# Jackson-D-Taylor/PINT

Measured on AMD Instinct MI355X. Metric: GLS fits/sec, 68-PSR x 10k-TOA synthetic PTA (whole node), higher is better.
Workload: dtype f64+dd; 1 GPU; pta68x10k GLSFitter.fit_toas(maxiter=1) incl. noise realisations (the 68-pulsar PTA, LPT-sharded over 1 rank(s)); npsr=68, ntoas=10000, K_cols_max=178, launch=direct, pipelines=2, parallelism=pulsar shards x1 (LPT, no data-path collective)

## Files before the change

### pint_amd/csrc/pint_hip.hip

```cpp
#include <hip/hip_runtime.h>
#include <hip/hip_ext.h>
#include <string>
#include <vector>
#include <cstring>
#include <cstdio>
#include <algorithm>
#include <array>
#include <utility>
#include <cmath>
#include <cstdlib>
#include <map>
#include <type_traits>
#include <mutex>
#include <functional>
#include <chrono>
#include "physics.hpp"
#include "ensemble.hpp"

using namespace pint;

typedef double double4_t __attribute__((ext_vector_type(4)));

__device__ __forceinline__ void rot(double& c, double& s, double c1, double s1) {
    const double cn = c * c1 - s * s1;
// ... 66 lines not shown
    const int32_t* fdj_index;
    const uint64_t *fdjmask, *fdjdmmask;
    int o_pw, npw, o_wave, nwave, sifunc, nifunc;
    const double *ifx_hi, *ifx_lo, *ify;
    const int32_t* dm_cls;
    const double* dme0;
    int ndmcls;
};

struct InstDev {
    int psr;
    int n;
    int K;
    int Kp;
    long toff;
    long roff;
    long moff;
    long goff;
    long soff;
    long coff;
    long cvoff;
    long eoff;
    long epoff;
    long ooff;
    long sdoff;
    long ddoff;
    long vgoff;
    long vboff;
    long xwoff;
    int self;
    int nrb;
    long rb0;
    int neb;
    long eb0;
    const pint_spec_t* spec;
    const ColRun* runs;
    int ts;
    int nrun;
};

struct GramView {
    const double* Gp;
    int Kp;
    const int32_t* cmap;
    const double* Sd;
    const double* DD;
    __device__ __forceinline__ double operator()(int i, int j) const {
        if (!cmap) {
            if (i > j) { int t = i; i = j; j = t; }
            return Gp[(long)i * Kp + j];
        }
        int a = cmap[i], b = cmap[j];
        if (a >= 0 && b >= 0) {
            if (a > b) { int t = a; a = b; b = t; }
            return Gp[(long)a * Kp + b];
        }
        if (a < 0 && b < 0) return a == b ? DD[-a - 1] : 0.0;
        if (a < 0) return Sd[(long)(-a - 1) * Kp + b];
        return Sd[(long)(-b - 1) * Kp + a];
    }
};

__device__ __forceinline__ GramView gram_view(const PsrDev& Pd, const InstDev& I, const double* Gpart, bool cmp,
                                              const double* Sd, const double* DD) {
    GramView g;
    g.Gp = Gpart + I.goff;
// ... 2318 lines not shown
        part[(long)blockIdx.x * 512 + e] = (red[e] + red[512 + e]) + (red[1024 + e] + red[1536 + e]);
}

__global__ __launch_bounds__(256) void k_trig_sum(const TrigJob* __restrict__ jobs, const double* __restrict__ part) {
    __shared__ double T[512];
    const TrigJob J = jobs[blockIdx.x];
    for (int e = threadIdx.x; e < 512; e += 256) {
        double v = 0.0;
        for (int b = 0; b < J.nb; b++) v += part[(long)(J.b0 + b) * 512 + e];
        T[e] = v;
    }
    __syncthreads();
    const int m = threadIdx.x & 63, a = m & 7, b = m >> 3, kind = threadIdx.x >> 6;
    if (kind < 2 && (kind == 1 || J.trigU)) {
        const double* D = T + kind * 256;
        double* o = kind ? J.trigW : J.trigU;
        o[m] = D[a * 16 + b] - D[(8 + a) * 16 + 8 + b];
        o[VTRIG + m] = D[(8 + a) * 16 + b] + D[a * 16 + 8 + b];
    }
}

struct GredArgs {
    int nsplit, nparts, compact, vb;
    double* Gpart;
    double* colsq;
    const double* Sdp;
    const double* dmxv;
    double* Sd;
    double* DD;
    double* DCS;
    const double* BFp;
};

__device__ __forceinline__ void gred_bin(const InstDev& I, const PsrDev& Pd, const GredArgs& g, int a, int lane) {
    const int Kp = Pd.Kpd, Kc = Pd.Kd, r0 = Pd.red0c, nsplit = g.nsplit;
    const int SW = Kc + 3;
    const int cnt = Pd.dptr[a + 1] - Pd.dptr[a];
    const long lo = cnt > 0 ? Pd.didx[Pd.dptr[a]] : 0, hi = lo + cnt;
    long per = (I.n + nsplit - 1) / nsplit;
    per = (per + 3) / 4 * 4;
    const int q0 = (int)(lo / per), q1 = cnt > 0 ? (int)((hi - 1) / per) : q0 - 1;
    const double* part = g.Sdp + I.vgoff + (long)(a % Pd.vns) * SW;
    constexpr int GRB_R = 4;
    const bool vbp = g.vb && Pd.vb;
    double dcs[2][2 * GW][2];
    bool use[2 * GW];
    long doff[2 * GW];
#pragma unroll
    for (int k = 0; k < 2 * GW; k++) {
        const int q = q0 + k / GW, w = k % GW;
        const long s0_ = (long)q * per, s1_ = min((long)I.n, s0_ + per), len = s1_ - s0_;
        const long QV = (len + VCH - 1) / VCH * 16;
        const long w0 = s0_ + w * QV, w1 = min(s1_, w0 + QV);
        use[k] = q <= q1 && !(w0 >= w1 || hi <= w0 || lo >= w1);
        doff[k] = I.vboff + (((long)q * GW + w) * Pd.vns + a % Pd.vns) * 128;
    }
    double xr[GRB_R], sr[GRB_R];
#pragma unroll
    for (int u = 0; u < GRB_R; u++) {
        const long i = lo + lane + 64 * u;
        xr[u] = i < hi ? g.dmxv[I.ooff + i] : 0.0;
        sr[u] = i < hi ? Pd.isig[i] : 0.0;
    }
#pragma unroll
    for (int t = 0; t < 2; t++) {
        const int c = lane + 64 * t;
        const bool fc = vbp && c >= r0 && c < Kc;
        int e0 = 0, e1 = 0;
        if (fc) {
            const int h = (c - r0) >> 1, k = h + 1, a_ = k & 7, cc = k >> 3;
            const bool isin = ((c - r0) & 1) == 0;
            e0 = isin ? (8 + a_) * 8 + cc : a_ * 8 + cc;
            e1 = isin ? a_ * 8 + 4 + cc : (8 + a_) * 8 + 4 + cc;
        }
#pragma unroll
        for (int k = 0; k < 2 * GW; k++) {
            const bool ld = c <= Kc && (fc ? use[k] : (k % GW == 0 && q0 + k / GW <= q1));
            dcs[t][k][0] = ld ? (fc ? g.BFp[doff[k] + e0] : part[(long)(q0 + k / GW) * Pd.vns * SW + c]) : 0.0;
            dcs[t][k][1] = (ld && fc) ? g.BFp[doff[k] + e1] : 0.0;
        }
    }
#pragma unroll
    for (int t = 0; t < 2; t++) {
        const int c = lane + 64 * t;
        if (c > Kc) break;
        double v = 0.0;
        if (vbp && c >= r0 && c < Kc) {
            const bool isin = ((c - r0) & 1) == 0;
            const double sg = isin ? 1.0 : -1.0;
#pragma unroll
            for (int k = 0; k < 2 * GW; k++)
                if (use[k]) v += dcs[t][k][0] + sg * dcs[t][k][1];
            for (int q = q0 + 2; q <= q1; q++) {
                const int h = (c - r0) >> 1, kk = h + 1, a_ = kk & 7, cc = kk >> 3;
                const int e0 = isin ? (8 + a_) * 8 + cc : a_ * 8 + cc;
                const int e1 = isin ? a_ * 8 + 4 + cc : (8 + a_) * 8 + 4 + cc;
                const long s0_ = (long)q * per, s1_ = min((long)I.n, s0_ + per), len = s1_ - s0_;
                const long QV = (len + VCH - 1) / VCH * 16;
                for (int w = 0; w < GW; w++) {
                    const long w0 = s0_ + w * QV, w1 = min(s1_, w0 + QV);
                    if (w0 >= w1 || hi <= w0 || lo >= w1) continue;
                    const double* D = g.BFp + I.vboff + (((long)q * GW + w) * Pd.vns + a % Pd.vns) * 128;
                    v += D[e0] + sg * D[e1];
                }
            }
        } else {
#pragma unroll
            for (int k = 0; k < 2; k++)
                if (q0 + k <= q1) v += dcs[t][k * GW][0];
            for (int q = q0 + 2; q <= q1; q++) v += part[(long)q * Pd.vns * SW + c];
        }
        g.Sd[I.sdoff + (long)a * Kp + c] = v;
    }
    for (int c = lane + 128; c <= Kc; c += 64) {
        double v = 0.0;
        if (vbp && c >= r0 && c < Kc) {
            const int h = (c - r0) >> 1, k = h + 1, a_ = k & 7, cc = k >> 3;
            const bool isin = ((c - r0) & 1) == 0;
            const int e0 = isin ? (8 + a_) * 8 + cc : a_ * 8 + cc;
            const int e1 = isin ? a_ * 8 + 4 + cc : (8 + a_) * 8 + 4 + cc;
            const double sg = isin ? 1.0 : -1.0;
            for (int q = q0; q <= q1; q++) {
                const long s0_ = (long)q * per, s1_ = min((long)I.n, s0_ + per), len = s1_ - s0_;
                const long QV = (len + VCH - 1) / VCH * 16;
                for (int w = 0; w < GW; w++) {
                    const long w0 = s0_ + w * QV, w1 = min(s1_, w0 + QV);
                    if (w0 >= w1 || hi <= w0 || lo >= w1) continue;
                    const double* D = g.BFp + I.vboff + (((long)q * GW + w) * Pd.vns + a % Pd.vns) * 128;
                    v += D[e0] + sg * D[e1];
                }
            }
        } else {
            for (int q = q0; q <= q1; q++) v += part[(long)q * Pd.vns * SW + c];
        }
        g.Sd[I.sdoff + (long)a * Kp + c] = v;
    }
    double q2 = 0.0, qw = 0.0;
#pragma unroll
    for (int u = 0; u < GRB_R; u++) {
        if (lo + lane + 64 * u < hi) {
            const double xx = xr[u], xw = xx * sr[u];
            q2 += xx * xx;
            qw += xw * xw;
        }
    }
    for (long i = lo + lane + 64 * GRB_R; i < hi; i += 64) {
        const double xx = g.dmxv[I.ooff + i], xw = xx * Pd.isig[i];
        q2 += xx * xx;
        qw += xw * xw;
    }
    q2 = wave_sum(q2);
    qw = wave_sum(qw);
    if (lane == 0) {
        g.DCS[I.ddoff + a] = q2;
        g.DD[I.ddoff + a] = qw;
    }
}

__device__ __forceinline__ void gred_elem(const InstDev& I, const PsrDev& Pd, const GredArgs& g, long e) {
    const bool cmp = g.compact && Pd.dsplit;
    const bool vg = cmp && Pd.vg;
    const int Kp = cmp ? Pd.Kpd : I.Kp, Kc = cmp ? Pd.Kd : I.K;
    const int r0 = Pd.red0c;
    const long KK = (long)Kp * Kp;
    if (e < KK) {
        const int i = (int)(e / Kp), j = (int)(e % Kp);
        if (i <= j) {
            double* G = g.Gpart + I.goff;
            if (vg && (j > Kc)) {
                G[e] = 0.0;
            } else if (vg && i >= r0 && j < Kc) {
                const double* C = Pd.trigW;
                const double* Sn = C + VTRIG;
                const int ha = (i - r0) / 2 + 1, sa = (i - r0) & 1;
                const int hb = (j - r0) / 2 + 1, sb = (j - r0) & 1;
                const int dm = ha > hb ? ha - hb : hb - ha, sm = ha + hb;
                const double sd = ha >= hb ? Sn[ha - hb] : -Sn[hb - ha];
                double v;
                if (sa == 0 && sb == 0) v = 0.5 * (C[dm] - C[sm]);
                else if (sa == 1 && sb == 1) v = 0.5 * (C[dm] + C[sm]);
                else if (sa == 0) v = 0.5 * (Sn[sm] + sd);
                else v = 0.5 * (Sn[sm] - sd);
                G[e] = v;
            } else {
                double a[8] = {G[e], 0.0, 0.0, 0.0, 0.0, 0.0, 0.0, 0.0};
                int q = 1;
                for (; q + 32 <= g.nparts; q += 32) {
                    double t[32];
#pragma unroll
                    for (int u = 0; u < 32; u++) t[u] = G[(long)(q + u) * KK + e];
#pragma unroll
                    for (int u = 0; u < 32; u++) a[u & 7] += t[u];
                }
                {
                    const int rem = g.nparts - q;
                    double t[31];
#pragma unroll
                    for (int u = 0; u < 31; u++) t[u] = u < rem ? G[(long)(q + u) * KK + e] : 0.0;
#pragma unroll
                    for (int r = 0; r < 3; r++)
                        if (8 * r + 8 <= rem) {
#pragma unroll
                            for (int u = 0; u < 8; u++) a[u] += t[8 * r + u];
                        }
#pragma unroll
                    for (int u = 0; u < 31; u++)
                        if (u >= (rem & ~7) && u < rem) a[0] += t[u];
                }
                G[e] = ((a[0] + a[1]) + (a[2] + a[3])) + ((a[4] + a[5]) + (a[6] + a[7]));
            }
        }
    }
    if (e < Kc) {
        double* cs = g.colsq + (I.coff + e) * g.nsplit;
        if (vg && e >= r0) {
            const double* U = Pd.trigU;
            const int h = (int)(e - r0) / 2 + 1;
            cs[0] = 0.5 * (U[0] + (((e - r0) & 1) ? U[2 * h] : -U[2 * h]));
        } else {
            double a[4] = {cs[0], 0.0, 0.0, 0.0};
            int q = 1;
            for (; q + 32 <= g.nsplit; q += 32) {
                double t[32];
#pragma unroll
                for (int u = 0; u < 32; u++) t[u] = cs[q + u];
#pragma unroll
                for (int u = 0; u < 32; u++) a[u & 3] += t[u];
            }
            {
                const int rem = g.nsplit - q;
                double t[31];
#pragma unroll
                for (int u = 0; u < 31; u++) t[u] = u < rem ? cs[q + u] : 0.0;
#pragma unroll
                for (int r = 0; r < 7; r++)
                    if (4 * r + 4 <= rem) {
#pragma unroll
                        for (int u = 0; u < 4; u++) a[u] += t[4 * r + u];
                    }
#pragma unroll
                for (int u = 0; u < 31; u++)
                    if (u >= (rem & ~3) && u < rem) a[0] += t[u];
            }
            cs[0] = (a[0] + a[1]) + (a[2] + a[3]);
        }
    }
}

__global__ __launch_bounds__(256) void k_greduce(const PsrDev* __restrict__ psrs, const InstDev* __restrict__ insts,
                                                 int nbg, GredArgs g) {
    WgTimer wgt_(WGT_GRED);
    const InstDev I = insts[blockIdx.y];
    const PsrDev& Pd = psrs[I.psr];
    const bool vg = g.compact && Pd.dsplit && Pd.vg;
    if ((int)blockIdx.x >= nbg) {
        const int a = (blockIdx.x - nbg) * 4 + (threadIdx.x >> 6);
        if (!vg || a >= Pd.ndc) return;
        gred_bin(I, Pd, g, a, threadIdx.x & 63);
        return;
    }
    gred_elem(I, Pd, g, (long)blockIdx.x * blockDim.x + threadIdx.x);
}

__device__ __forceinline__ bool ones_virtual(const pint_spec_t& S) { return S.o_PHOFF >= 0 && !S.wb_noones; }

__global__ __launch_bounds__(64) void k_onesrow(const PsrDev* __restrict__ psrs, const InstDev* __restrict__ insts,
                                                const double* __restrict__ esum, const double* __restrict__ eD,
                                                const double* __restrict__ eW, const double* __restrict__ eC,
                                                int compact, const double* __restrict__ M, double* __restrict__ ones) {
    const InstDev I = insts[blockIdx.x];
    const PsrDev& Pd = psrs[I.psr];
    const pint_spec_t& S = *Pd.spec;
    if (!ones_virtual(S) || !(S.nred > 0 || Pd.nep > 0)) return;
    const bool cmp = compact && Pd.dsplit;
    const int R = 2 * S.nred, jd = 2 * S.dmn0;
    if (jd < R) {
        const int n = I.n;
        const double* Fb = M + I.moff + (long)(cmp ? Pd.red0c : S.ncol) * n;
        for (int j = jd; j < R; j++) {
            double acc = 0.0;
            for (int i = threadIdx.x; i < n; i += 64) {
                const double is = Pd.isig[i];
                acc += Fb[(long)j * n + i] * (is * is);
            }
            acc = wave_sum(acc);
            if (threadIdx.x == 0) {
                for (int e = 0; e < Pd.nep; e++) {
                    const double w = eW[I.epoff + e];
                    acc -= w * esum_col(Pd, I, esum, eC, cmp, e, S.ncol + j) / eD[I.epoff + e];
                }
                ones[I.coff + j] = acc;
            }
        }
    }
// ... 3002 lines not shown
    bool psrs_dirty = false;
    PsrDev* d_psrs = nullptr;
    int npsr_dev = 0;
    int ninst = 0;
    std::vector<InstDev> inst;
    InstDev* d_inst = nullptr;
    InstDev* d_inst_sorted = nullptr;
    InstDev* d_inst_sorted_c = nullptr;
    InstDev* d_inst_sorted_v = nullptr;
    bool sorted_alias[3] = {false, false, false};
    double* d_gridspec = nullptr;
    std::vector<KpGroup> kp_groups, kp_groups_c, kp_groups_v;
    int vgram = 1;
    int vbin = 1;
    int wbfit = 0;
    int gv_pair = 1;
    int maxn = 0;
    int max_ts = 0;
    int resid12 = 1;
    int prep_lanes = 1;
    int fuse_r2 = 1;
    bool r2_pending = false;
    int resid_path = 0;
    int eval_path = 0;
    int eval_kinds = 0;
    bool grid_valid = false;
    std::vector<double> grid_spec_host;
    int grid_psr = -1;
    std::vector<int32_t> points_toff;
    bool points_valid = false;
    struct EnsState* ens = nullptr;
    long grid_opts = 0;
    int small = 1;
    int schur = 1;
    int evalb_wpe = 3;
    int la_chol = 1;
    int solve_w8 = 1;
    int eval0_wpe = 1;
    int eval_wpe = 3;
    int n_vg = 0;
    bool any_dmx_rows = false;
    double *d_TSp = nullptr, *d_TS = nullptr;
    double* d_Sdp = nullptr;
    double* d_BFp = nullptr;
    int vb_on = 0;
    double* d_xw = nullptr;
    int cov_defer = 1;
    bool cov_pending = false;
    int cov_mode = 0;
    size_t cov_lds = 0;
    bool ic_valid = false;
    bool phases_valid = false;
    bool no_events = false;
    int timing_mask = 0xff;
    int timing_every = 1;
    long gram_calls = 0;
    static constexpr int NSLOT = PINT_NSLOT;
    hipGraph_t graph_s[NSLOT] = {};
    hipGraphExec_t graph_exec_s[NSLOT] = {};
    bool capturing = false;
    int* d_blk_inst = nullptr;
    int* d_blk_row0 = nullptr;
    int* d_rblk_inst = nullptr;
    double* d_rpart = nullptr;
    double* d_epart = nullptr;
    int efz = 0;
// ... 532 lines not shown
        return;
    }
    std::lock_guard<std::mutex> lk(g_stream_mu);
    g_stream_pool[role][device][g_stream_rank[s]] = s;
}

pint_ctx* pint_ctx_create(int device) {
    pint_ctx* ctx = new pint_ctx();
    ctx->device = device;
    if (hipSetDevice(device) != hipSuccess) {
        ctx->err = "hipSetDevice failed";
        return ctx;
    }
    {
        int ncu = 0;
        if (hipDeviceGetAttribute(&ncu, hipDeviceAttributeMultiprocessorCount, device) == hipSuccess && ncu > 0) ctx->ncu = ncu;
    }
    ctx->stream = stream_get(device, STREAM_KERNEL);
    ctx->cstream = stream_get(device, STREAM_COPY);
    const unsigned evf = hipEventDisableTiming |
                         ((getenv("PINT_EV_SYSTEM") && atoi(getenv("PINT_EV_SYSTEM"))) ? 0u : hipEventReleaseToDevice);
    hipEventCreateWithFlags(&ctx->ev_solved, evf);
    hipEventCreateWithFlags(&ctx->ev_copied, evf);
    hipEventCreateWithFlags(&ctx->ev_noise, evf);
    if (getenv("PINT_SERIAL") && atoi(getenv("PINT_SERIAL"))) ctx->sstream = ctx->stream;
    else ctx->sstream = stream_get(device, STREAM_SIDE);
    ctx->no_events = getenv("PINT_NO_EVENTS") && atoi(getenv("PINT_NO_EVENTS"));
    ctx->eval_merge = getenv("PINT_EVAL_MERGE") ? atoi(getenv("PINT_EVAL_MERGE")) : 3;
    ctx->vbin = getenv("PINT_VBIN") ? (atoi(getenv("PINT_VBIN")) ? 1 : 0) : 1;
    ctx->cov_defer = getenv("PINT_COV_DEFER") ? atoi(getenv("PINT_COV_DEFER")) : 1;
    ctx->eval_wpe = getenv("PINT_EVAL_WPE") ? atoi(getenv("PINT_EVAL_WPE")) : 3;
    ctx->gv_pair = getenv("PINT_GV_PAIR") ? atoi(getenv("PINT_GV_PAIR")) : 1;
    ctx->schur = getenv("PINT_SCHUR") ? atoi(getenv("PINT_SCHUR")) : 1;
    ctx->fuse_r2 = getenv("PINT_FUSE_R2") ? atoi(getenv("PINT_FUSE_R2")) : 1;
    ctx->eval0_wpe = getenv("PINT_EVAL0_WPE") ? atoi(getenv("PINT_EVAL0_WPE")) : 1;
    ctx->prep_lanes = getenv("PINT_PREP_LANES") ? atoi(getenv("PINT_PREP_LANES")) : 1;
    ctx->resid12 = getenv("PINT_RESID12") ? atoi(getenv("PINT_RESID12")) : 1;
    ctx->evalb_wpe = getenv("PINT_EVALB_WPE") ? atoi(getenv("PINT_EVALB_WPE")) : 3;
    ctx->la_chol = getenv("PINT_LA_CHOL") ? atoi(getenv("PINT_LA_CHOL")) : 1;
    ctx->solve_w8 = getenv("PINT_SOLVE_W8") ? atoi(getenv("PINT_SOLVE_W8")) : 1;
    ctx->efuse = getenv("PINT_EFUSE") ? atoi(getenv("PINT_EFUSE")) : 1;
    ctx->lane_solve = getenv("PINT_LANE_SOLVE") ? atoi(getenv("PINT_LANE_SOLVE")) : 1;
    ctx->spin_eval = getenv("PINT_SPIN_EVAL") ? atoi(getenv("PINT_SPIN_EVAL")) : 1;
    hipEventCreateWithFlags(&ctx->ev_gram, evf);
    hipEventCreateWithFlags(&ctx->ev_sigma, evf);
    for (int sl = 0; sl < pint_ctx::NSLOT; sl++) {
        hipEventCreateWithFlags(&ctx->ev_done[sl], evf);
        hipEventCreateWithFlags(&ctx->ev_cdone[sl], hipEventDisableTiming);
    }
    hipMalloc(&ctx->d_status_slots, pint_ctx::NSLOT * sizeof(int));
    hipMemset(ctx->d_status_slots, 0, pint_ctx::NSLOT * sizeof(int));
    ctx->d_status = ctx->d_status_slots;
    hipHostMalloc(&ctx->h_status, pint_ctx::NSLOT * sizeof(int), hipHostMallocDefault);
    if (ctx->h_status)
        for (int sl = 0; sl < pint_ctx::NSLOT; sl++) ctx->h_status[sl] = 0;
    return ctx;
}

const char* pint_last_error(pint_ctx* ctx) { return ctx ? ctx->err.c_str() : "null context"; }

struct GramOrder {
    std::vector<KpGroup> groups;
    std::vector<int> order;
    bool ident;
};
struct VgChoice {
// ... 146 lines not shown
        const PsrDev& d = ph.dev;
        VgChoice& v = out[pi];
        v = VgChoice{0, 0, d.vns, d.vkp, false};
        if (!vg_ok(ctx, ph)) continue;
        const int wt = d.red0c + 1, R = d.Kd - d.red0c;
        const int ntr = first_ntr(ph, std::max((wt + 15) / 16, std::min(3, force_ntr)), nsplit);
        if (!ntr) continue;
        v.vg = 1;
        v.vns = 16 * ntr - wt;
        v.vkp = (16 * ntr + R + 15) / 16 * 16;
        v.reslot = ph.dslot_ns != v.vns;
        if (ctx->vbin && v.vkp <= 96 && v.vns >= 16) v.vg = v.vb = vb_rows_ok(ph, nsplit) ? 1 : 0;
    }
    return out;
}

static void layout_instances(const pint_ctx* ctx, int ninst, const int32_t* inst_psr, BatchLayout& L) {
    const int nsplit = L.nsplit;
    std::vector<int> bti[PINT_NBLK], btr[PINT_NBLK];
    L.inst.resize(ninst);
    for (int k = 0; k < ninst; k++) {
        const int p = inst_psr[k];
        const PsrHost& ph = ctx->psrs[p];
        const VgChoice& v = L.vg[p];
        InstDev& I = L.inst[k];
        I.psr = p;
        I.n = ph.n;
        I.spec = nullptr;
        I.runs = nullptr;
        I.ts = ph.spec.tstride;
        I.nrun = ph.dev.nrun;
        I.K = ph.K;
        I.Kp = ph.dev.Kp;
        I.toff = L.tot_table;
        I.roff = L.tot_rows;
        I.moff = L.tot_m;
        I.goff = L.tot_g;
        I.soff = L.tot_s;
        I.coff = L.tot_c;
        I.cvoff = L.tot_cv;
        I.eoff = L.tot_e;
        I.epoff = L.tot_ep;
        I.ooff = L.tot_out;
        I.sdoff = L.tot_sd;
        I.ddoff = L.tot_dd;
        I.vgoff = L.vgoff;
        I.vboff = L.vboff;
        I.xwoff = L.xwoff;
        if (v.vg) {
            L.vgoff += (long)nsplit * v.vns * (ph.dev.Kd + 3);
            if (v.vb) L.vboff += (long)nsplit * GW * v.vns * 128;
            L.n_vg++;
        } else if (ph.dev.dsplit) {
            L.any_dmx_rows = true;
        }
        if (ph.dev.dsplit) {
            L.tot_sd += (long)ph.dev.ndc * ph.dev.Kpd;
            L.tot_dd += ph.dev.ndc;
            const long nbd = (ph.dev.Kd + 15) / 16, nbk = (ph.dev.ndc + 15) / 16;
            L.xwoff += (nbd * (nbd + 1) / 2 + nbd * nbk) * 256 + (nbd + 3 * nbk) * 16 + schur_xw_extra(nbd, nbk);
            L.max_ndc = std::max(L.max_ndc, ph.dev.ndc);
        }
        I.self = k;
        I.rb0 = (long)L.rblk_inst.size();
        I.nrb = std::max(1, (ph.n + RES_RB - 1) / RES_RB);
        for (int b = 0; b < I.nrb; b++) L.rblk_inst.push_back(k);
// ... 1667 lines not shown
using GramVKernel = decltype(&k_gram_v<1, 1, false>);
struct GramVEntry {
    int key;
    GramVKernel kern[2];
};
template <int R, int C>
constexpr GramVEntry gram_v_entry() {
    return {10 * (R - 1) + C, {k_gram_v<R, C, false>, k_gram_v<R, C, true>}};
}
constexpr GramVEntry GRAM_V_KERNELS[PINT_PLAN_MAXVKEY] = {
    gram_v_entry<1, 1>(), gram_v_entry<1, 2>(), gram_v_entry<1, 3>(), gram_v_entry<1, 4>(), gram_v_entry<1, 5>(),
    gram_v_entry<1, 6>(), gram_v_entry<1, 7>(), gram_v_entry<2, 2>(), gram_v_entry<2, 3>(), gram_v_entry<2, 4>(),
    gram_v_entry<2, 5>(), gram_v_entry<2, 6>(), gram_v_entry<2, 7>(), gram_v_entry<3, 3>(), gram_v_entry<3, 4>(),
    gram_v_entry<3, 5>(), gram_v_entry<3, 6>(), gram_v_entry<3, 7>()};
extern "C" {

constexpr size_t FIT_LDS = 160 * 1024;
static inline int nb16(int k) { return (k + 15) / 16; }

struct FitShape {
    int Kn;
    int Ks_rest;
    int Ks_all;
    int ndmx;
    bool dmx_fit;
    int nbd, nbk;
    size_t lds_x;
    int maxKd;
    bool any_gather;
    bool noise;
    int nbs_sig;
    bool ones;
    int maxKp;
    bool all_vg;
    int maxts;
};

static FitShape fit_shape(const pint_ctx* ctx, int mode) {
    FitShape s{};
    s.dmx_fit = s.all_vg = true;
    s.maxKp = 16;
    int kn_sig = 0;
    for (int pi : ctx->upsr) {
        const PsrHost& ph = ctx->psrs[pi];
        const pint_spec_t& sp = ph.spec;
        const PsrDev& pd = ph.dev;
        const bool ds = ctx->m_compact && pd.dsplit;
        const bool noisy = mode == 1 && (sp.nred > 0 || pd.nep > 0);
        const int kn = mode == 1 ? 2 * sp.nred + 1 : 0, ks = mode == 0 ? sp.ncol : ph.K;
        s.Kn = std::max(s.Kn, kn);
        s.Ks_all = std::max(s.Ks_all, ks);
        if (noisy) s.noise = true, kn_sig = std::max(kn_sig, kn);
        if (noisy && sp.o_PHOFF >= 0 && !sp.wb_noones) s.ones = true;
        s.maxKp = std::max(s.maxKp, ds ? pd.Kpd : pd.Kp);
        s.all_vg = s.all_vg && ds && pd.vg;
        s.maxts = std::max(s.maxts, sp.tstride);
        if (!ds) {
            s.Ks_rest = std::max(s.Ks_rest, ks);
            continue;
        }
        s.ndmx++;
        const int nbd = nb16(mode == 0 ? pd.red0c : pd.Kd), nbk = nb16(pd.ndc), nbs = nb16(kn);
        const int blk = nbd * (nbd + 1) / 2 + nbd * nbk;
        if (blk > SD_MAXBLK || nbd > 17 || nbs > BS_MAXNB) s.dmx_fit = false;
        s.lds_x = std::max(s.lds_x, sizeof(double) * ((size_t)std::max(blk, nbs * (nbs + 1) / 2) * 256 +
                                                      (size_t)(5 * nbd + 6 * nbk) * 16));
        s.nbd = std::max(s.nbd, nbd);
        s.nbk = std::max(s.nbk, nbk);
        s.maxKd = std::max(s.maxKd, pd.Kd);
        if (!pd.dcontig) s.any_gather = true;
    }
    s.nbs_sig = nb16(kn_sig);
    return s;
}

struct FitPlan {
    const char* err;
    pint_plan_t pub;
    int mode, nparts, skip;
    bool ecorr;
    bool ones, vgp;
    bool ext_t, gram_mark;
    size_t lds_rows;
    struct GramGroup {
        GramKernel kern, kern_ecorr;
        size_t lds;
    } gram[GMAXT_ALL + 1];
    struct GramVGroup {
        GramVKernel kern;
        uint32_t lds;
    } gramv[PINT_PLAN_MAXVKEY];
    int nbg;
    size_t lds_s, lds_x, lds_dyn, lds_col;
    bool xw, pre, w8, apply_tail;
    int mnb;
    size_t lds_schur;
    int ldsw, ldsw1;
};

static const GramVEntry* gram_v_kernels(int key) {
    for (const GramVEntry& e : GRAM_V_KERNELS)
        if (e.key == key) return &e;
    return nullptr;
}

static FitPlan plan_refused(const char* why) {
    FitPlan p{};
    p.err = why;
    return p;
}

static FitPlan plan_fit_step(const pint_ctx* ctx, int mode, bool apply_req, bool sampled) {
    const bool cmp = ctx->m_compact;
    if (ctx->wbfit) {
        if (!cmp) return plan_refused("wideband fit: the DM rows need the compact fit layout (pint_eval with want_M = 2)");
        for (int pi : ctx->upsr) {
            const pint_spec_t& sp = ctx->psrs[pi].spec;
            if (!ctx->psrs[pi].dev.wb) continue;
            if (!ctx->psrs[pi].dev.dsplit)
                return plan_refused("wideband fit: a pulsar with wideband DM data is not on the compact DMX layout "
                                    "(>= 8 free DMX bins, no TOA in two free bins, every ECORR epoch within one bin)");
            int m = 0;
            for (int c = 0; c < sp.ncol; c++)
                m += (sp.col_kind[c] == PINT_COL_DM || sp.col_kind[c] == PINT_COL_ZERO || sp.col_kind[c] == PINT_COL_NESW);
            if (m > WB_MAXC)
// ... 27 lines not shown
        return plan_refused("Woodbury Sigma too large for the LDS factorisation");
    if (cmp && ctx->max_ndc > 0 && ctx->any_dmx_rows) {
        pl.dmx_rows = 1;
        pl.dmx = s.any_gather;
        pl.ecorr_dmx = p.ecorr;
        p.lds_rows = sizeof(double) * (DMX_RS * ((s.maxKd + 2) | 1) + 2 * DMX_RS);
    }
    const std::vector<KpGroup>& groups = cmp ? ctx->kp_groups_c : ctx->kp_groups;
    p.vgp = cmp && ctx->n_vg > 0;
    const bool gram_t = !ctx->no_events && !ctx->capturing && ((ctx->timing_mask >> 6) & 1) && sampled;
    p.ext_t = gram_t && p.vgp && groups.empty() && !ctx->kp_groups_v.empty();
    p.gram_mark = sampled && !p.ext_t;
    for (size_t g = 0; g < groups.size(); g++) {
        const int T = groups[g].T, Te = std::max(T, 1);
        if ((int)g > GMAXT_ALL || T < 0 || T > GMAXT_ALL) return plan_refused("Kp out of range");
        const int CH = gram_ch(Te);
        p.gram[g] = {T ? GRAM_KERNELS[0][T - 1] : nullptr, p.ecorr ? GRAM_KERNELS[1][Te - 1] : nullptr,
                     sizeof(double) * ((size_t)groups[g].maxKp * (CH + 2) + CH)};
        if (T) pl.gram_t_mask |= 1 << T;
        else pl.gram_s = 1;
        if (p.ecorr) pl.gram_ecorr = 1, pl.gram_t_mask |= 1 << Te;
    }
    for (size_t g = 0; p.vgp && g < ctx->kp_groups_v.size(); g++) {
        const KpGroup& kg = ctx->kp_groups_v[g];
        const GramVEntry* e = gram_v_kernels(kg.T);
        if (g >= PINT_PLAN_MAXVKEY || !e) return plan_refused("k_gram_v layout out of range");
        const int vb = (ctx->vb_on && kg.T % 10 <= 6) ? 1 : 0;
        const size_t lds = sizeof(double) * std::max<size_t>((size_t)GVB * (kg.maxKp + (ctx->vb_on && kg.maxKp <= 96 ? 33 : 17)) * (VCH + 2),
                                                             std::max(GW * VTG * 256, GW * 256 + 256));
        p.gramv[g] = {e->kern[vb], (uint32_t)lds};
        pl.vkey[pl.nvkey] = kg.T;
        pl.vkey_vb[pl.nvkey++] = vb;
    }
    pl.greduce = p.nparts > 1 || p.vgp;
    p.nbg = (s.maxKp * s.maxKp + 255) / 256;
    pl.wb_gram = ctx->wbfit && cmp;
    if (p.skip) {
        p.xw = ctx->d_xw && (ctx->cov_defer == 2 || (ctx->cov_defer == 1 && (ctx->ninst >= 16 || ctx->lazy)));
        p.lds_dyn = pl.fuse_sigma ? std::max(p.lds_x, p.lds_s) : p.lds_x;
        const size_t lds_apply = p.lds_x + apply_tail_lds(s.maxts);
        if (apply_req && all_dmx && !pl.side_sigma && !pl.do_sigma && s.all_vg && lds_apply <= FIT_LDS - 512) {
            p.apply_tail = true;
            p.lds_dyn = std::max(p.lds_dyn, lds_apply);
        }
        p.pre = p.xw && ctx->schur && s.nbd > 0;
        p.mnb = s.nbd * (s.nbd + 1) / 2;
        p.lds_schur = schur_lds(s.nbk);
        p.w8 = ctx->solve_w8 && s.nbd <= 8 && (!pl.fuse_sigma || s.nbs_sig <= 9);
        pl.solve_dmx_waves = p.w8 ? 8 : 16;
        pl.schur = p.pre;
        pl.cov_deferred = p.xw;
    }
    p.ldsw = nbx * (nbx + 1) / 2 * 256 + 2 * 16 * nbx;
    p.ldsw1 = p.ldsw + 3 * 16 * nbx;
    if (all_dmx) pl.solve = PINT_PLAN_SOLVE_NONE;
    else if (col_solve) pl.solve = PINT_PLAN_SOLVE_COLUMN;
    else if (nbx <= 1 && ctx->small && ctx->lane_solve && !p.skip && Ks <= 8)
        pl.solve = Ks <= 4 ? PINT_PLAN_SOLVE_LANES4 : PINT_PLAN_SOLVE_LANES8;
    else if (nbx <= 2 && ctx->small) pl.solve = PINT_PLAN_SOLVE_BLK1;
    else pl.solve = nbx <= 5 ? PINT_PLAN_SOLVE_BLK4 : PINT_PLAN_SOLVE_BLK16;
    return p;
}

static int launch_ecorr(pint_ctx* ctx, const FitPlan& p) {
    if (!p.ecorr) return PINT_OK;
    if (any_copy_pend(ctx)) {
        HIPCHK(hipStreamWaitEvent(ctx->stream, ctx->ev_copied, 0));
        clear_copy_pend(ctx);
// ... 51 lines not shown
                                   ctx->d_G, ctx->d_colsq);
        }
    }
    HIPCHK(hipGetLastError());
    return PINT_OK;
}

static int launch_gram_v(pint_ctx* ctx, const FitPlan& p) {
    if (p.ext_t)
        for (int i : {12, 13})
            if (!ctx->ev[i]) HIPCHK(hipEventCreate(&ctx->ev[i]));
    const GvResid gvr{ctx->d_rp, ctx->d_ftay, ctx->d_rpart, ctx->r2_pending ? 1 : 0, ctx->efz ? ctx->d_epart : nullptr};
    const size_t ng = p.vgp ? ctx->kp_groups_v.size() : 0;
    for (size_t g = 0; g < ng; g++) {
        const KpGroup& kg = ctx->kp_groups_v[g];
        hipEvent_t e0 = (p.ext_t && g == 0) ? ctx->ev[12] : nullptr;
        hipEvent_t e1 = (p.ext_t && g + 1 == ng) ? ctx->ev[13] : nullptr;
        hipExtLaunchKernelGGL(p.gramv[g].kern, dim3(ctx->nsplit, kg.count), dim3(GW * 64), p.gramv[g].lds, ctx->stream,
                              e0, e1, 0u, (const PsrDev*)ctx->d_psrs, (const InstDev*)(ctx->d_inst_sorted_v + kg.first),
                              (const double*)ctx->d_M, (const double*)ctx->d_rt, (const double*)ctx->d_dmxv, ctx->nsplit,
                              ctx->d_G, ctx->d_Sdp, ctx->d_colsq, ctx->d_TSp, ctx->d_BFp, ctx->gvdbg, gvr);
    }
    if (p.ext_t) ctx->rec[12] = ctx->rec[13] = true;
    else if (p.gram_mark) record(ctx, 13);
    HIPCHK(hipGetLastError());
    return PINT_OK;
}

static int launch_greduce(pint_ctx* ctx, const FitPlan& p) {
    if (!p.pub.greduce) return PINT_OK;
    const GredArgs gra{ctx->nsplit, p.nparts, ctx->m_compact, ctx->vb_on, ctx->d_G, ctx->d_colsq, ctx->d_Sdp,
                       ctx->d_dmxv, ctx->d_Sd, ctx->d_DD, ctx->d_DCS, ctx->d_BFp};
    record(ctx, 14);
    hipLaunchKernelGGL(k_greduce, dim3(p.nbg + (p.vgp ? (ctx->max_ndc + 3) / 4 : 0), ctx->ninst), dim3(256), 0,
                       ctx->stream, ctx->d_psrs, ctx->d_inst, p.nbg, gra);
    HIPCHK(hipGetLastError());
    record(ctx, 15);
    return PINT_OK;
}

static int launch_wb_gram(pint_ctx* ctx, const FitPlan& p) {
    if (!p.pub.wb_gram) return PINT_OK;
    if (int rc = ensure_ic_solar_wind(ctx)) return rc;
    hipLaunchKernelGGL(k_wb_gram, dim3(ctx->ninst), dim3(256), 0, ctx->stream, ctx->d_psrs, ctx->d_inst, ctx->d_tables,
                       ctx->d_ic, ctx->nsplit, ctx->d_G, ctx->d_colsq, ctx->d_Sd, ctx->d_DD, ctx->d_DCS);
    HIPCHK(hipGetLastError());
    return PINT_OK;
}

static int launch_side_sigma(pint_ctx* ctx, const FitPlan& p) {
    if (!p.pub.side_sigma) return PINT_OK;
    HIPCHK(hipEventRecord(ctx->ev_gram, ctx->stream));
    HIPCHK(hipStreamWaitEvent(ctx->sstream, ctx->ev_gram, 0));
    const int nw = p.pub.sigma_waves;
    const auto kern = nw == 4 ? k_sigma<4> : k_sigma<16>;
    hipLaunchKernelGGL(kern, dim3(ctx->ninst), dim3(nw * 64), p.lds_s, ctx->sstream, ctx->d_psrs, ctx->d_inst,
                       ctx->d_tables, ctx->d_G, ctx->m_compact, ctx->d_Sd, ctx->d_DD, ctx->d_sigL, ctx->d_status,
                       p.ones ? ctx->d_ones : nullptr);
    HIPCHK(hipGetLastError());
    HIPCHK(hipEventRecord(ctx->ev_sigma, ctx->sstream));
    ctx->sigma_pending = true;
    return PINT_OK;
}

static int launch_solve_dmx(pint_ctx* ctx, const FitPlan& p, double lam) {
    ctx->cov_pending = false;
    if (!p.skip) return PINT_OK;
// ... 1889 lines not shown
```

Before: 223,300 fits/s.

## Add tiled triangular Gram-reduce kernel with multi-bin workgroups

Result: no change. 225,100 fits/s (median of 2 runs) (+0.8%).

```diff
diff --git a/pint_amd/csrc/pint_hip.hip b/pint_amd/csrc/pint_hip.hip
--- a/pint_amd/csrc/pint_hip.hip
+++ b/pint_amd/csrc/pint_hip.hip
@@ -122,6 +122,7 @@
     int nrb;
     long rb0;
     int neb;
+    unsigned gred;
     long eb0;
     const pint_spec_t* spec;
     const ColRun* runs;
@@ -2506,109 +2507,95 @@
     const double* BFp;
 };
 
-__device__ __forceinline__ void gred_bin(const InstDev& I, const PsrDev& Pd, const GredArgs& g, int a, int lane) {
-    const int Kp = Pd.Kpd, Kc = Pd.Kd, r0 = Pd.red0c, nsplit = g.nsplit;
-    const int SW = Kc + 3;
-    const int cnt = Pd.dptr[a + 1] - Pd.dptr[a];
-    const long lo = cnt > 0 ? Pd.didx[Pd.dptr[a]] : 0, hi = lo + cnt;
-    long per = (I.n + nsplit - 1) / nsplit;
-    per = (per + 3) / 4 * 4;
-    const int q0 = (int)(lo / per), q1 = cnt > 0 ? (int)((hi - 1) / per) : q0 - 1;
-    const double* part = g.Sdp + I.vgoff + (long)(a % Pd.vns) * SW;
-    constexpr int GRB_R = 4;
-    const bool vbp = g.vb && Pd.vb;
-    double dcs[2][2 * GW][2];
-    bool use[2 * GW];
-    long doff[2 * GW];
+constexpr int GRB_R = 4;
+constexpr int GRB_WG = 16;
+
+struct GredBin {
+    int lo, hi;
+    int q0, q1;
+    unsigned use;
+};
+__device__ __forceinline__ int gred_per(int n, int nsplit) { return ((n + nsplit - 1) / nsplit + 3) / 4 * 4; }
+__device__ __forceinline__ bool gred_quarter(int n, int per, int q, int w, int lo, int hi) {
+    const int s0_ = q * per, s1_ = min(n, s0_ + per), len = s1_ - s0_;
+    const int QV = (len + VCH - 1) / VCH * 16;
+    const int w0 = s0_ + w * QV, w1 = min(s1_, w0 + QV);
+    return !(w0 >= w1 || hi <= w0 || lo >= w1);
+}
+__device__ __forceinline__ GredBin gred_bin_geo(const InstDev& I, const PsrDev& Pd, int nsplit, int a) {
+    GredBin B;
+    const int p0 = Pd.dptr[a], cnt = Pd.dptr[a + 1] - p0;
+    B.lo = cnt > 0 ? Pd.didx[p0] : 0;
+    B.hi = B.lo + cnt;
+    const int per = gred_per(I.n, nsplit);
+    B.q0 = B.lo / per;
+    B.q1 = cnt > 0 ? (B.hi - 1) / per : B.q0 - 1;
+    B.use = 0;
 #pragma unroll
     for (int k = 0; k < 2 * GW; k++) {
-        const int q = q0 + k / GW, w = k % GW;
-        const long s0_ = (long)q * per, s1_ = min((long)I.n, s0_ + per), len = s1_ - s0_;
-        const long QV = (len + VCH - 1) / VCH * 16;
-        const long w0 = s0_ + w * QV, w1 = min(s1_, w0 + QV);
-        use[k] = q <= q1 && !(w0 >= w1 || hi <= w0 || lo >= w1);
-        doff[k] = I.vboff + (((long)q * GW + w) * Pd.vns + a % Pd.vns) * 128;
-    }
-    double xr[GRB_R], sr[GRB_R];
+        const int q = B.q0 + k / GW;
+        if (q <= B.q1 && gred_quarter(I.n, per, q, k % GW, B.lo, B.hi)) B.use |= 1u << k;
+    }
+    return B;
+}
+
+__device__ __forceinline__ double gred_sd_col(const InstDev& I, const PsrDev& Pd, const GredArgs& g, const GredBin& B,
+                                              int a, int c) {
+    const int Kc = Pd.Kd, r0 = Pd.red0c, SW = Kc + 3, slot = a % Pd.vns;
+    const double* part = g.Sdp + I.vgoff + (long)slot * SW;
+    const bool fc = g.vb && Pd.vb && c >= r0 && c < Kc;
+    const int q0 = B.q0, q1 = B.q1;
+    int e0 = 0, e1 = 0;
+    const bool isin = ((c - r0) & 1) == 0;
+    if (fc) {
+        const int h = (c - r0) >> 1, k = h + 1, a_ = k & 7, cc = k >> 3;
+        e0 = isin ? (8 + a_) * 8 + cc : a_ * 8 + cc;
+        e1 = isin ? a_ * 8 + 4 + cc : (8 + a_) * 8 + 4 + cc;
+    }
+    const double sg = isin ? 1.0 : -1.0;
+    double d[2 * GW][2];
+#pragma unroll
+    for (int k = 0; k < 2 * GW; k++) {
+        const int q = q0 + k / GW;
+        const bool ld = fc ? ((B.use >> k) & 1) != 0 : (k % GW == 0 && q <= q1);
+        const long doff = I.vboff + (((long)q * GW + k % GW) * Pd.vns + slot) * 128;
+        d[k][0] = ld ? (fc ? g.BFp[doff + e0] : part[(long)q * Pd.vns * SW + c]) : 0.0;
+        d[k][1] = (ld && fc) ? g.BFp[doff + e1] : 0.0;
+    }
+    double v = 0.0;
+    if (fc) {
+#pragma unroll
+        for (int k = 0; k < 2 * GW; k++)
+            if ((B.use >> k) & 1) v += d[k][0] + sg * d[k][1];
+        if (q0 + 2 <= q1) {
+            const int per = gred_per(I.n, g.nsplit);
+            for (int q = q0 + 2; q <= q1; q++)
+                for (int w = 0; w < GW; w++) {
+                    if (!gred_quarter(I.n, per, q, w, B.lo, B.hi)) continue;
+                    const double* D = g.BFp + I.vboff + (((long)q * GW + w) * Pd.vns + slot) * 128;
+                    v += D[e0] + sg * D[e1];
+                }
+        }
+    } else {
+#pragma unroll
+        for (int k = 0; k < 2; k++)
+            if (q0 + k <= q1) v += d[k * GW][0];
+        for (int q = q0 + 2; q <= q1; q++) v += part[(long)q * Pd.vns * SW + c];
+    }
+    return v;
+}
+
+__device__ __forceinline__ void gred_dd_load(const InstDev& I, const PsrDev& Pd, const GredArgs& g, int lo, int hi,
+                                             int lane, double (&xr)[GRB_R], double (&sr)[GRB_R]) {
 #pragma unroll
     for (int u = 0; u < GRB_R; u++) {
-        const long i = lo + lane + 64 * u;
+        const int i = lo + lane + 64 * u;
         xr[u] = i < hi ? g.dmxv[I.ooff + i] : 0.0;
         sr[u] = i < hi ? Pd.isig[i] : 0.0;
     }
-#pragma unroll
-    for (int t = 0; t < 2; t++) {
-        const int c = lane + 64 * t;
-        const bool fc = vbp && c >= r0 && c < Kc;
-        int e0 = 0, e1 = 0;
-        if (fc) {
-            const int h = (c - r0) >> 1, k = h + 1, a_ = k & 7, cc = k >> 3;
-            const bool isin = ((c - r0) & 1) == 0;
-            e0 = isin ? (8 + a_) * 8 + cc : a_ * 8 + cc;
-            e1 = isin ? a_ * 8 + 4 + cc : (8 + a_) * 8 + 4 + cc;
-        }
-#pragma unroll
-        for (int k = 0; k < 2 * GW; k++) {
-            const bool ld = c <= Kc && (fc ? use[k] : (k % GW == 0 && q0 + k / GW <= q1));
-            dcs[t][k][0] = ld ? (fc ? g.BFp[doff[k] + e0] : part[(long)(q0 + k / GW) * Pd.vns * SW + c]) : 0.0;
-            dcs[t][k][1] = (ld && fc) ? g.BFp[doff[k] + e1] : 0.0;
-        }
-    }
-#pragma unroll
-    for (int t = 0; t < 2; t++) {
-        const int c = lane + 64 * t;
-        if (c > Kc) break;
-        double v = 0.0;
-        if (vbp && c >= r0 && c < Kc) {
-            const bool isin = ((c - r0) & 1) == 0;
-            const double sg = isin ? 1.0 : -1.0;
-#pragma unroll
-            for (int k = 0; k < 2 * GW; k++)
-                if (use[k]) v += dcs[t][k][0] + sg * dcs[t][k][1];
-            for (int q = q0 + 2; q <= q1; q++) {
-                const int h = (c - r0) >> 1, kk = h + 1, a_ = kk & 7, cc = kk >> 3;
-                const int e0 = isin ? (8 + a_) * 8 + cc : a_ * 8 + cc;
-                const int e1 = isin ? a_ * 8 + 4 + cc : (8 + a_) * 8 + 4 + cc;
-                const long s0_ = (long)q * per, s1_ = min((long)I.n, s0_ + per), len = s1_ - s0_;
-                const long QV = (len + VCH - 1) / VCH * 16;
-                for (int w = 0; w < GW; w++) {
-                    const long w0 = s0_ + w * QV, w1 = min(s1_, w0 + QV);
-                    if (w0 >= w1 || hi <= w0 || lo >= w1) continue;
-                    const double* D = g.BFp + I.vboff + (((long)q * GW + w) * Pd.vns + a % Pd.vns) * 128;
-                    v += D[e0] + sg * D[e1];
-                }
-            }
-        } else {
-#pragma unroll
-            for (int k = 0; k < 2; k++)
-                if (q0 + k <= q1) v += dcs[t][k * GW][0];
-            for (int q = q0 + 2; q <= q1; q++) v += part[(long)q * Pd.vns * SW + c];
-        }
-        g.Sd[I.sdoff + (long)a * Kp + c] = v;
-    }
-    for (int c = lane + 128; c <= Kc; c += 64) {
-        double v = 0.0;
-        if (vbp && c >= r0 && c < Kc) {
-            const int h = (c - r0) >> 1, k = h + 1, a_ = k & 7, cc = k >> 3;
-            const bool isin = ((c - r0) & 1) == 0;
-            const int e0 = isin ? (8 + a_) * 8 + cc : a_ * 8 + cc;
-            const int e1 = isin ? a_ * 8 + 4 + cc : (8 + a_) * 8 + 4 + cc;
-            const double sg = isin ? 1.0 : -1.0;
-            for (int q = q0; q <= q1; q++) {
-                const long s0_ = (long)q * per, s1_ = min((long)I.n, s0_ + per), len = s1_ - s0_;
-                const long QV = (len + VCH - 1) / VCH * 16;
-                for (int w = 0; w < GW; w++) {
-                    const long w0 = s0_ + w * QV, w1 = min(s1_, w0 + QV);
-                    if (w0 >= w1 || hi <= w0 || lo >= w1) continue;
-                    const double* D = g.BFp + I.vboff + (((long)q * GW + w) * Pd.vns + a % Pd.vns) * 128;
-                    v += D[e0] + sg * D[e1];
-                }
-            }
-        } else {
-            for (int q = q0; q <= q1; q++) v += part[(long)q * Pd.vns * SW + c];
-        }
-        g.Sd[I.sdoff + (long)a * Kp + c] = v;
-    }
+}
+__device__ __forceinline__ void gred_dd_sum(const InstDev& I, const PsrDev& Pd, const GredArgs& g, int a, int lo,
+                                            int hi, int lane, const double (&xr)[GRB_R], const double (&sr)[GRB_R]) {
     double q2 = 0.0, qw = 0.0;
 #pragma unroll
     for (int u = 0; u < GRB_R; u++) {
@@ -2618,7 +2605,7 @@
             qw += xw * xw;
         }
     }
-    for (long i = lo + lane + 64 * GRB_R; i < hi; i += 64) {
+    for (int i = lo + lane + 64 * GRB_R; i < hi; i += 64) {
         const double xx = g.dmxv[I.ooff + i], xw = xx * Pd.isig[i];
         q2 += xx * xx;
         qw += xw * xw;
@@ -2631,94 +2618,98 @@
     }
 }
 
-__device__ __forceinline__ void gred_elem(const InstDev& I, const PsrDev& Pd, const GredArgs& g, long e) {
-    const bool cmp = g.compact && Pd.dsplit;
-    const bool vg = cmp && Pd.vg;
-    const int Kp = cmp ? Pd.Kpd : I.Kp, Kc = cmp ? Pd.Kd : I.K;
+__device__ __forceinline__ void gred_bin(const InstDev& I, const PsrDev& Pd, const GredArgs& g, int a, int lane) {
+    const GredBin B = gred_bin_geo(I, Pd, g.nsplit, a);
+    double xr[GRB_R], sr[GRB_R];
+    gred_dd_load(I, Pd, g, B.lo, B.hi, lane, xr, sr);
+    for (int c = lane; c <= Pd.Kd; c += 64) g.Sd[I.sdoff + (long)a * Pd.Kpd + c] = gred_sd_col(I, Pd, g, B, a, c);
+    gred_dd_sum(I, Pd, g, a, B.lo, B.hi, lane, xr, sr);
+}
+
+__device__ __forceinline__ double gred_sum_parts(const double* G, long e, long KK, int nparts) {
+    double a[8] = {G[e], 0.0, 0.0, 0.0, 0.0, 0.0, 0.0, 0.0};
+    int q = 1;
+    for (; q + 32 <= nparts; q += 32) {
+        double t[32];
+#pragma unroll
+        for (int u = 0; u < 32; u++) t[u] = G[(long)(q + u) * KK + e];
+#pragma unroll
+        for (int u = 0; u < 32; u++) a[u & 7] += t[u];
+    }
+    {
+        const int rem = nparts - q;
+        double t[31];
+#pragma unroll
+        for (int u = 0; u < 31; u++) t[u] = u < rem ? G[(long)(q + u) * KK + e] : 0.0;
+#pragma unroll
+        for (int r = 0; r < 3; r++)
+            if (8 * r + 8 <= rem) {
+#pragma unroll
+                for (int u = 0; u < 8; u++) a[u] += t[8 * r + u];
+            }
+#pragma unroll
+        for (int u = 0; u < 31; u++)
+            if (u >= (rem & ~7) && u < rem) a[0] += t[u];
+    }
+    return ((a[0] + a[1]) + (a[2] + a[3])) + ((a[4] + a[5]) + (a[6] + a[7]));
+}
+
+__device__ __forceinline__ double gred_fourier(const PsrDev& Pd, int i, int j) {
     const int r0 = Pd.red0c;
-    const long KK = (long)Kp * Kp;
-    if (e < KK) {
-        const int i = (int)(e / Kp), j = (int)(e % Kp);
-        if (i <= j) {
-            double* G = g.Gpart + I.goff;
-            if (vg && (j > Kc)) {
-                G[e] = 0.0;
-            } else if (vg && i >= r0 && j < Kc) {
-                const double* C = Pd.trigW;
-                const double* Sn = C + VTRIG;
-                const int ha = (i - r0) / 2 + 1, sa = (i - r0) & 1;
-                const int hb = (j - r0) / 2 + 1, sb = (j - r0) & 1;
-                const int dm = ha > hb ? ha - hb : hb - ha, sm = ha + hb;
-                const double sd = ha >= hb ? Sn[ha - hb] : -Sn[hb - ha];
-                double v;
-                if (sa == 0 && sb == 0) v = 0.5 * (C[dm] - C[sm]);
-                else if (sa == 1 && sb == 1) v = 0.5 * (C[dm] + C[sm]);
-                else if (sa == 0) v = 0.5 * (Sn[sm] + sd);
-                else v = 0.5 * (Sn[sm] - sd);
-                G[e] = v;
-            } else {
-                double a[8] = {G[e], 0.0, 0.0, 0.0, 0.0, 0.0, 0.0, 0.0};
-                int q = 1;
-                for (; q + 32 <= g.nparts; q += 32) {
-                    double t[32];
-#pragma unroll
-                    for (int u = 0; u < 32; u++) t[u] = G[(long)(q + u) * KK + e];
-#pragma unroll
-                    for (int u = 0; u < 32; u++) a[u & 7] += t[u];
-                }
-                {
-                    const int rem = g.nparts - q;
-                    double t[31];
-#pragma unroll
-                    for (int u = 0; u < 31; u++) t[u] = u < rem ? G[(long)(q + u) * KK + e] : 0.0;
-#pragma unroll
-                    for (int r = 0; r < 3; r++)
-                        if (8 * r + 8 <= rem) {
-#pragma unroll
-                            for (int u = 0; u < 8; u++) a[u] += t[8 * r + u];
-                        }
-#pragma unroll
-                    for (int u = 0; u < 31; u++)
-                        if (u >= (rem & ~7) && u < rem) a[0] += t[u];
-                }
-                G[e] = ((a[0] + a[1]) + (a[2] + a[3])) + ((a[4] + a[5]) + (a[6] + a[7]));
+    const double* C = Pd.trigW;
+    const double* Sn = C + VTRIG;
+    const int ha = ((i - r0) >> 1) + 1, sa = (i - r0) & 1;
+    const int hb = ((j - r0) >> 1) + 1, sb = (j - r0) & 1;
+    const int dm = ha > hb ? ha - hb : hb - ha, sm = ha + hb;
+    const double sd = ha >= hb ? Sn[ha - hb] : -Sn[hb - ha];
+    if (sa == 0 && sb == 0) return 0.5 * (C[dm] - C[sm]);
+    if (sa == 1 && sb == 1) return 0.5 * (C[dm] + C[sm]);
+    if (sa == 0) return 0.5 * (Sn[sm] + sd);
+    return 0.5 * (Sn[sm] - sd);
+}
+
+__device__ __forceinline__ void gred_elem(const PsrDev& Pd, double* G, bool vg, int Kc, long KK, int nparts, int i,
+                                          int j, long e) {
+    if (vg && j > Kc) G[e] = 0.0;
+    else if (vg && i >= Pd.red0c && j < Kc) G[e] = gred_fourier(Pd, i, j);
+    else G[e] = gred_sum_parts(G, e, KK, nparts);
+}
+__device__ __forceinline__ int gred_nparts(const GredArgs& g, bool vg) { return vg ? g.nsplit : g.nparts; }
+
+__device__ __forceinline__ void gred_colsq(const InstDev& I, const PsrDev& Pd, const GredArgs& g, bool vg, int c) {
+    const int r0 = Pd.red0c;
+    double* cs = g.colsq + (I.coff + c) * g.nsplit;
+    if (vg && c >= r0) {
+        const double* U = Pd.trigU;
+        const int h = ((c - r0) >> 1) + 1;
+        cs[0] = 0.5 * (U[0] + (((c - r0) & 1) ? U[2 * h] : -U[2 * h]));
+        return;
+    }
+    double a[4] = {cs[0], 0.0, 0.0, 0.0};
+    int q = 1;
+    for (; q + 32 <= g.nsplit; q += 32) {
+        double t[32];
+#pragma unroll
+        for (int u = 0; u < 32; u++) t[u] = cs[q + u];
+#pragma unroll
+        for (int u = 0; u < 32; u++) a[u & 3] += t[u];
+    }
+    {
+        const int rem = g.nsplit - q;
+        double t[31];
+#pragma unroll
+        for (int u = 0; u < 31; u++) t[u] = u < rem ? cs[q + u] : 0.0;
+#pragma unroll
+        for (int r = 0; r < 7; r++)
+            if (4 * r + 4 <= rem) {
+#pragma unroll
+                for (int u = 0; u < 4; u++) a[u] += t[4 * r + u];
             }
-        }
-    }
-    if (e < Kc) {
-        double* cs = g.colsq + (I.coff + e) * g.nsplit;
-        if (vg && e >= r0) {
-            const double* U = Pd.trigU;
-            const int h = (int)(e - r0) / 2 + 1;
-            cs[0] = 0.5 * (U[0] + (((e - r0) & 1) ? U[2 * h] : -U[2 * h]));
-        } else {
-            double a[4] = {cs[0], 0.0, 0.0, 0.0};
-            int q = 1;
-            for (; q + 32 <= g.nsplit; q += 32) {
-                double t[32];
-#pragma unroll
-                for (int u = 0; u < 32; u++) t[u] = cs[q + u];
-#pragma unroll
-                for (int u = 0; u < 32; u++) a[u & 3] += t[u];
-            }
-            {
-                const int rem = g.nsplit - q;
-                double t[31];
-#pragma unroll
-                for (int u = 0; u < 31; u++) t[u] = u < rem ? cs[q + u] : 0.0;
-#pragma unroll
-                for (int r = 0; r < 7; r++)
-                    if (4 * r + 4 <= rem) {
-#pragma unroll
-                        for (int u = 0; u < 4; u++) a[u] += t[4 * r + u];
-                    }
-#pragma unroll
-                for (int u = 0; u < 31; u++)
-                    if (u >= (rem & ~3) && u < rem) a[0] += t[u];
-            }
-            cs[0] = (a[0] + a[1]) + (a[2] + a[3]);
-        }
-    }
+#pragma unroll
+        for (int u = 0; u < 31; u++)
+            if (u >= (rem & ~3) && u < rem) a[0] += t[u];
+    }
+    cs[0] = (a[0] + a[1]) + (a[2] + a[3]);
 }
 
 __global__ __launch_bounds__(256) void k_greduce(const PsrDev* __restrict__ psrs, const InstDev* __restrict__ insts,
@@ -2726,14 +2717,87 @@
     WgTimer wgt_(WGT_GRED);
     const InstDev I = insts[blockIdx.y];
     const PsrDev& Pd = psrs[I.psr];
-    const bool vg = g.compact && Pd.dsplit && Pd.vg;
+    const bool cmp = g.compact && Pd.dsplit;
+    const bool vg = cmp && Pd.vg;
     if ((int)blockIdx.x >= nbg) {
         const int a = (blockIdx.x - nbg) * 4 + (threadIdx.x >> 6);
         if (!vg || a >= Pd.ndc) return;
         gred_bin(I, Pd, g, a, threadIdx.x & 63);
         return;
     }
-    gred_elem(I, Pd, g, (long)blockIdx.x * blockDim.x + threadIdx.x);
+    const int Kp = cmp ? Pd.Kpd : I.Kp, Kc = cmp ? Pd.Kd : I.K;
+    const long KK = (long)Kp * Kp, e = (long)blockIdx.x * blockDim.x + threadIdx.x;
+    if (e < KK) {
+        const int i = (int)(e / Kp), j = (int)(e % Kp);
+        if (i <= j) gred_elem(Pd, g.Gpart + I.goff, vg, Kc, KK, gred_nparts(g, vg), i, j, e);
+    }
+    if (e < Kc) gred_colsq(I, Pd, g, vg, (int)e);
+}
+
+__device__ __forceinline__ void tri_decode(int p, int& i, int& j);
+
+__global__ __launch_bounds__(256) void k_greduce_t(const PsrDev* __restrict__ psrs, const InstDev* __restrict__ insts,
+                                                   int ntg, GredArgs g) {
+    __shared__ int sb[GRB_WG][5];
+    WgTimer wgt_(WGT_GRED);
+    const InstDev& I = insts[blockIdx.y];
+    const int x = blockIdx.x;
+    if (x >= ntg) {
+        const int a0 = (x - ntg) * GRB_WG, nbin = g.compact ? (int)(I.gred >> 16) : 0;
+        if (a0 >= nbin) return;
+        const PsrDev& Pd = psrs[I.psr];
+        const int nb = min(GRB_WG, nbin - a0), tid = threadIdx.x, wave = tid >> 6, lane = tid & 63;
+        if (tid < nb) {
+            const GredBin B = gred_bin_geo(I, Pd, g.nsplit, a0 + tid);
+            sb[tid][0] = B.lo;
+            sb[tid][1] = B.hi;
+            sb[tid][2] = B.q0;
+            sb[tid][3] = B.q1;
+            sb[tid][4] = (int)B.use;
+        }
+        __syncthreads();
+        double xr[4][GRB_R], sr[4][GRB_R];
+#pragma unroll
+        for (int b = 0; b < 4; b++) {
+            const int bb = 4 * wave + b;
+            gred_dd_load(I, Pd, g, bb < nb ? sb[bb][0] : 0, bb < nb ? sb[bb][1] : 0, lane, xr[b], sr[b]);
+        }
+        const unsigned W = Pd.Kd + 1, nitem = nb * W;
+        for (unsigned it = tid; it < nitem; it += 256) {
+            const unsigned b = it / W, c = it - b * W;
+            const GredBin B{sb[b][0], sb[b][1], sb[b][2], sb[b][3], (unsigned)sb[b][4]};
+            g.Sd[I.sdoff + (long)(a0 + b) * Pd.Kpd + c] = gred_sd_col(I, Pd, g, B, a0 + b, c);
+        }
+#pragma unroll
+        for (int b = 0; b < 4; b++) {
+            const int bb = 4 * wave + b;
+            if (bb < nb) gred_dd_sum(I, Pd, g, a0 + bb, sb[bb][0], sb[bb][1], lane, xr[b], sr[b]);
+        }
+        return;
+    }
+    const int Kp = g.compact ? (int)(I.gred & 0xffff) : I.Kp, nt = Kp >> 4, ntile = nt * (nt + 1) / 2;
+    if (x > ntile) return;
+    const PsrDev& Pd = psrs[I.psr];
+    const bool cmp = g.compact && Pd.dsplit;
+    const bool vg = cmp && Pd.vg;
+    const int Kc = cmp ? Pd.Kd : I.K;
+    if (x == ntile) {
+        for (int c = threadIdx.x; c < Kc; c += 256) gred_colsq(I, Pd, g, vg, c);
+        return;
+    }
+    int Ib, Jb;
+    tri_decode(x, Jb, Ib);
+    Ib = __builtin_amdgcn_readfirstlane(Ib);
+    Jb = __builtin_amdgcn_readfirstlane(Jb);
+    const int i = 16 * Ib + (threadIdx.x >> 4), j = 16 * Jb + (threadIdx.x & 15);
+    if (i > j) return;
+    const int r0 = Pd.red0c;
+    const long KK = (long)Kp * Kp, e = (long)i * Kp + j;
+    double* G = g.Gpart + I.goff;
+    if (vg && 16 * Ib >= r0 && 16 * Jb + 15 < Kc) G[e] = gred_fourier(Pd, i, j);
+    else if (vg && 16 * Jb > Kc) G[e] = 0.0;
+    else if (!vg || (16 * Ib + 15 < r0 && 16 * Jb + 15 <= Kc)) G[e] = gred_sum_parts(G, e, KK, gred_nparts(g, vg));
+    else gred_elem(Pd, G, vg, Kc, KK, gred_nparts(g, vg), i, j, e);
 }
 
 __device__ __forceinline__ bool ones_virtual(const pint_spec_t& S) { return S.o_PHOFF >= 0 && !S.wb_noones; }
@@ -5802,6 +5866,7 @@
     struct EnsState* ens = nullptr;
     long grid_opts = 0;
     int small = 1;
+    int gred = 1;
     int schur = 1;
     int evalb_wpe = 3;
     int la_chol = 1;
@@ -6400,6 +6465,7 @@
     ctx->eval_wpe = getenv("PINT_EVAL_WPE") ? atoi(getenv("PINT_EVAL_WPE")) : 3;
     ctx->gv_pair = getenv("PINT_GV_PAIR") ? atoi(getenv("PINT_GV_PAIR")) : 1;
     ctx->schur = getenv("PINT_SCHUR") ? atoi(getenv("PINT_SCHUR")) : 1;
+    ctx->gred = getenv("PINT_GRED") ? atoi(getenv("PINT_GRED")) : 1;
     ctx->fuse_r2 = getenv("PINT_FUSE_R2") ? atoi(getenv("PINT_FUSE_R2")) : 1;
     ctx->eval0_wpe = getenv("PINT_EVAL0_WPE") ? atoi(getenv("PINT_EVAL0_WPE")) : 1;
     ctx->prep_lanes = getenv("PINT_PREP_LANES") ? atoi(getenv("PINT_PREP_LANES")) : 1;
@@ -6612,6 +6678,8 @@
         I.nrun = ph.dev.nrun;
         I.K = ph.K;
         I.Kp = ph.dev.Kp;
+        I.gred = (unsigned)((ph.dev.dsplit ? ph.dev.Kpd : ph.dev.Kp) & 0xffff) |
+                 ((unsigned)((v.vg && ph.dev.dsplit ? ph.dev.ndc : 0) & 0xffff) << 16);
         I.toff = L.tot_table;
         I.roff = L.tot_rows;
         I.moff = L.tot_m;
@@ -8345,13 +8413,14 @@
     int nbs_sig;
     bool ones;
     int maxKp;
+    bool gred_fit;
     bool all_vg;
     int maxts;
 };
 
 static FitShape fit_shape(const pint_ctx* ctx, int mode) {
     FitShape s{};
-    s.dmx_fit = s.all_vg = true;
+    s.dmx_fit = s.all_vg = s.gred_fit = true;
     s.maxKp = 16;
     int kn_sig = 0;
     for (int pi : ctx->upsr) {
@@ -8366,6 +8435,7 @@
         if (noisy) s.noise = true, kn_sig = std::max(kn_sig, kn);
         if (noisy && sp.o_PHOFF >= 0 && !sp.wb_noones) s.ones = true;
         s.maxKp = std::max(s.maxKp, ds ? pd.Kpd : pd.Kp);
+        if (pd.Kp > 0xffff || pd.Kpd > 0xffff || pd.ndc > 0xffff) s.gred_fit = false;
         s.all_vg = s.all_vg && ds && pd.vg;
         s.maxts = std::max(s.maxts, sp.tstride);
         if (!ds) {
@@ -8404,6 +8474,7 @@
         uint32_t lds;
     } gramv[PINT_PLAN_MAXVKEY];
     int nbg;
+    int nbb;
     size_t lds_s, lds_x, lds_dyn, lds_col;
     bool xw, pre, w8, apply_tail;
     int mnb;
@@ -8497,8 +8568,10 @@
         pl.vkey[pl.nvkey] = kg.T;
         pl.vkey_vb[pl.nvkey++] = vb;
     }
-    pl.greduce = p.nparts > 1 || p.vgp;
-    p.nbg = (s.maxKp * s.maxKp + 255) / 256;
+    pl.greduce = (p.nparts > 1 || p.vgp) ? (ctx->gred && s.gred_fit ? 2 : 1) : 0;
+    const int ntk = s.maxKp / 16;
+    p.nbg = pl.greduce == 2 ? ntk * (ntk + 1) / 2 + 1 : (s.maxKp * s.maxKp + 255) / 256;
+    p.nbb = !p.vgp ? 0 : (pl.greduce == 2 ? (ctx->max_ndc + GRB_WG - 1) / GRB_WG : (ctx->max_ndc + 3) / 4);
     pl.wb_gram = ctx->wbfit && cmp;
     if (p.skip) {
         p.xw = ctx->d_xw && (ctx->cov_defer == 2 || (ctx->cov_defer == 1 && (ctx->ninst >= 16 || ctx->lazy)));
@@ -8616,7 +8689,7 @@
     const GredArgs gra{ctx->nsplit, p.nparts, ctx->m_compact, ctx->vb_on, ctx->d_G, ctx->d_colsq, ctx->d_Sdp,
                        ctx->d_dmxv, ctx->d_Sd, ctx->d_DD, ctx->d_DCS, ctx->d_BFp};
     record(ctx, 14);
-    hipLaunchKernelGGL(k_greduce, dim3(p.nbg + (p.vgp ? (ctx->max_ndc + 3) / 4 : 0), ctx->ninst), dim3(256), 0,
+    hipLaunchKernelGGL(p.pub.greduce == 2 ? k_greduce_t : k_greduce, dim3(p.nbg + p.nbb, ctx->ninst), dim3(256), 0,
                        ctx->stream, ctx->d_psrs, ctx->d_inst, p.nbg, gra);
     HIPCHK(hipGetLastError());
     record(ctx, 15);
```
